# jordi-adell/mcarray

Measured on AMD Instinct MI355X. Metric: STFT frames/sec, 8-mic GCC-PHAT + SRP-PHAT(361) + delay-and-sum beamform @48kHz/1024-pt, higher is better.
Workload: dtype f32 (SRP operands adaptive); 1 GPU; BASELINE configs[2] geometry (8-mic ULA 0.04 m, 48 kHz, N=1024, hop 512, 361 angles, 1 source, no power floor), 8 arrays x 4096 frames per GPU per step; channel rows padded by 64 floats; arrays_per_gpu=8, frames_per_array=4096, srp_precision=adaptive, parallelism=arrays sharded over 1 GPU(s), all_gather of DOA bins+prob

## Files before the change

### mcarray_amd/csrc/api.hip

```cpp
#include "../../include/mcarray_hip.h"
#include "fft1024c.h"
#include "kernels.h"
#include "knobs.h"
#include "stage.h"

#include <chrono>
#include <cmath>
#include <cstdio>
#include <cstdlib>
#include <cstring>
#include <string>
#include <thread>
#include <vector>

using namespace mca;

namespace {

std::string g_create_error;

struct TimedEvent { int id; hipEvent_t a, b; };

}

// ... 1639 lines not shown
           (c->prec == MCA_HIP_SRP_ADAPTIVE || c->prec == MCA_HIP_SRP_FP16) && c->cfg.gcc_weighting != MCA_HIP_GCC_NONE;
}

static int steer_pass_frames(const mca_hip_ctx *c, int n_arrays, int n_frames)
{
    const long long cap = ws_max_bytes(c) / ((long long)n_arrays * STEER_ROW * (long long)sizeof(float2));
    return (int)std::max<long long>(1, std::min<long long>(n_frames, cap));
}

static void steer_policy_begin(mca_hip_ctx *c)
{
    const unsigned long long s = c->steer_seq + 1;
    if (!c->h_steer || c->steer_lost || s <= FB_LAG) return;
    const unsigned long long r = s - FB_LAG;
    if (r <= c->steer_seq_seen) return;
    const unsigned long long *slot = c->h_steer + 2 * ((r - 1) % FB_RING);
    const auto t0 = std::chrono::steady_clock::now();
    while (__atomic_load_n(&slot[1], __ATOMIC_ACQUIRE) != r) {
        if (std::chrono::duration_cast<std::chrono::milliseconds>(std::chrono::steady_clock::now() - t0).count() > FB_WAIT_MS) { c->steer_lost = true; c->steer_spec = true; return; }
        std::this_thread::yield();
    }
    c->steer_seq_seen = r;
    c->steer_spec = __atomic_load_n(&slot[0], __ATOMIC_RELAXED) * STEER_MISS_DEN <= c->steer_call_frames[(r - 1) % FB_RING] * STEER_MISS_NUM;
}

static int steer_prepare(mca_hip_ctx *c, int n_arrays, int n_frames)
{
    if (!c->d_steer_rows) {
        const size_t na = (size_t)c->cfg.max_arrays;
        HIP_TRY(c, hipMalloc((void **)&c->d_steer_rows, (size_t)(c->D + 1) * 4 * 64 * sizeof(float4)));
        HIP_TRY(c, hipMalloc((void **)&c->d_steer_q, (size_t)(c->D + 1) * c->M * 8 * sizeof(float2)));
        HIP_TRY(c, hipMalloc((void **)&c->d_steer_nyq, (size_t)(c->D + 1) * c->M * sizeof(float)));
        HIP_TRY(c, hipMalloc((void **)&c->d_steer_pred, na * sizeof(int)));
        HIP_TRY(c, hipMalloc((void **)&c->d_steer_miss, 3 * sizeof(unsigned long long)));
        if (hipHostMalloc((void **)&c->h_steer, FB_RING * 16, hipHostMallocDefault) == hipSuccess) std::memset(c->h_steer, 0, FB_RING * 16); else { c->h_steer = nullptr; (void)hipGetLastError(); }
        HIP_TRY(c, hipMalloc((void **)&c->d_steer_tail, 2 * na * FFT_H * sizeof(float)));
        HIP_TRY(c, hipMemset(c->d_steer_pred, 0xff, na * sizeof(int)));
        HIP_TRY(c, hipMemset(c->d_steer_miss, 0, 3 * sizeof(unsigned long long)));
        const double unit = (double)c->cfg.sample_rate / (double)FFT_N / 346.1;
        hipLaunchKernelGGL(k_steer_table, dim3(c->D + 1, 4), dim3(64), 0, nullptr, c->d_steer_rows, c->d_steer_q, c->d_steer_nyq, c->d_grid, c->d_micx, c->M, unit);
        HIP_TRY(c, hipGetLastError());
        HIP_TRY(c, hipDeviceSynchronize());
    }
    const size_t rows = (size_t)n_arrays * steer_pass_frames(c, n_arrays, n_frames);
    if (rows > c->steer_Y_rows) {
        HIP_TRY(c, hipDeviceSynchronize());
        if (c->d_steer_Y) (void)hipFree(c->d_steer_Y);
        c->d_steer_Y = nullptr; c->steer_Y_rows = 0;
        HIP_TRY(c, hipMalloc((void **)&c->d_steer_Y, rows * STEER_ROW * sizeof(float2)));
        c->steer_Y_rows = rows;
    }
    return MCA_HIP_OK;
}

static int steer_reserve(mca_hip_ctx *c, int n_arrays, int n_frames) { return steer_applies(c) ? steer_prepare(c, n_arrays, n_frames) : MCA_HIP_OK; }

static int steer_separate(mca_hip_ctx *c, const float *pcm, long long array_stride, long long mic_stride, int n_arrays, int n_frames,
                          const int *doa_bin, float *out_pcm, hipStream_t st)
{
    const size_t a0 = (size_t)c->a0;
    const int pf = steer_pass_frames(c, n_arrays, n_frames);
    const bool fused = c->steer_fused_now && pf == n_frames;
    const size_t smem = (size_t)(F1K_TWORDS + 4 * F1K_SCRATCH) * sizeof(float2);
    float *tails[2] = {c->d_steer_tail, c->d_steer_tail + (size_t)c->cfg.max_arrays * FFT_H};
    time_begin(c, MCA_HIP_K_BEAMFORM, st);
    int pass = 0;
    for (int f0 = 0; f0 < n_frames; f0 += pf, ++pass) {
        const int f1 = std::min(n_frames, f0 + pf), np = f1 - f0;
        const bool last = f1 == n_frames;
        SteerPatchArgs pa{};
        pa.pcm = pcm; pa.array_stride = array_stride; pa.mic_stride = mic_stride; pa.n_arrays = n_arrays; pa.n_frames = n_frames; pa.f0 = f0; pa.f1 = f1;
        pa.window = c->d_window; pa.doa_bin = doa_bin; pa.all = fused ? 0 : 1; pa.miss = c->d_steer_miss;
        pa.bf.rows = c->d_steer_rows; pa.bf.q = c->d_steer_q; pa.bf.nyq = c->d_steer_nyq; pa.bf.pred = c->d_steer_pred + a0; pa.bf.Y = c->d_steer_Y;
        pa.y_f0 = f0; pa.y_frames = fused ? n_frames : np;
        hipLaunchKernelGGL(k_steer_patch, dim3(std::min(STEER_PATCH_WGS, (np + 3) / 4)), dim3(256), smem, st, pa);
        SteerSynthArgs sy{};
        sy.Y = c->d_steer_Y; sy.n_frames = n_frames; sy.f0 = f0; sy.f1 = f1; sy.y_f0 = pa.y_f0; sy.y_frames = pa.y_frames;
        sy.ft = 16;
        while (sy.ft > 2 && (long long)n_arrays * ((np + sy.ft - 1) / sy.ft) < 1024) sy.ft >>= 1;
        sy.out = out_pcm;
        sy.tail_in = pass == 0 ? c->d_tail[c->tail_cur] + a0 * FFT_H : tails[(pass - 1) & 1];
        sy.tail_out = last ? c->d_tail[c->tail_cur ^ 1] + a0 * FFT_H : tails[pass & 1];
        sy.doa_bin = doa_bin; sy.pred_out = last ? c->d_steer_pred + a0 : nullptr;
        if (last && c->h_steer) { sy.report = c->h_steer + 2 * (c->steer_seq % FB_RING); sy.seq = c->steer_seq + 1; sy.miss_total = c->d_steer_miss; }
        const int runs = (np + sy.ft - 1) / sy.ft;
        hipLaunchKernelGGL(k_steer_synth, dim3((runs + 3) / 4, n_arrays), dim3(256), smem, st, sy);
    }
    time_end(c, st);
    HIP_TRY(c, hipGetLastError());
    c->steer_call_frames[c->steer_seq % FB_RING] = (unsigned long long)n_arrays * n_frames; ++c->steer_seq;
    c->steer_frames_total += (unsigned long long)n_arrays * n_frames;
    if (fused) ++c->steer_fused_calls;
    return MCA_HIP_OK;
}

static int separate_impl(mca_hip_ctx *c, const float *pcm, long long array_stride, long long mic_stride,
                         int n_arrays, int n_frames, const float *doa_rad, float *out_pcm, hipStream_t st, const int *doa_bin = nullptr)
{
    const size_t a0 = (size_t)c->a0;
    if (doa_bin && c->d_bftab && c->n2048 && (reinterpret_cast<uintptr_t>(out_pcm) & 7) == 0) {
        BeamformWaveArgs wa{};
        wa.pcm = pcm; wa.array_stride = array_stride; wa.mic_stride = mic_stride;
        wa.M = c->M; wa.n_pairs = c->M; wa.n_frames = n_frames; wa.S = c->S;
        wa.ft = 16;
        for (int ft = 2; ft <= 64; ++ft)
            if ((long long)n_arrays * c->S * ((n_frames + 4 * ft - 2) / (4 * ft - 1)) <= 2LL * c->n_cu) { wa.ft = ft; break; }
        wa.window = c->d_window; wa.doa_bin = doa_bin; wa.table = c->d_bftab; wa.out = out_pcm;
        wa.tail_in = c->d_tail[c->tail_cur] + a0 * c->S * c->H; wa.tail_out = c->d_tail[c->tail_cur ^ 1] + a0 * c->S * c->H;
        const int wgs = (n_frames + 4 * wa.ft - 2) / (4 * wa.ft - 1);
        const size_t smem_w = (size_t)(F1K_TWORDS + 4 * F1K_SCRATCH + 4 * 512) * sizeof(float2);
        time_begin(c, MCA_HIP_K_BEAMFORM, st);
        hipLaunchKernelGGL(k_beamform_wave_2048, dim3(wgs, n_arrays, c->S), dim3(256), smem_w, st, wa);
        time_end(c, st);
        HIP_TRY(c, hipGetLastError());
        return MCA_HIP_OK;
    }
    if (doa_bin && c->d_bftab && wave_beamformer_applies(c)) {
        BeamformWaveArgs wa{};
        wa.pcm = pcm; wa.array_stride = array_stride; wa.mic_stride = mic_stride;
// ... 959 lines not shown
    return MCA_HIP_OK;
}

static int drain_events(mca_hip_ctx *c)
{
    for (auto &e : c->events) {
        HIP_TRY(c, hipEventSynchronize(e.b));
        float ms = 0.f;
        HIP_TRY(c, hipEventElapsedTime(&ms, e.a, e.b));
        c->t_ms[e.id] += ms; c->t_launches[e.id] += 1;
        c->pool.push_back(e.a); c->pool.push_back(e.b);
    }
    c->events.clear();
    return MCA_HIP_OK;
}

int mca_hip_get_timing(mca_hip_ctx *c, int kernel_id, int *launches, double *total_ms)
{
    if (!c || kernel_id < 0 || kernel_id >= MCA_HIP_K_COUNT) return MCA_HIP_ERR_INVALID_ARGUMENT;
    int rc = drain_events(c);
    if (rc) return rc;
    if (launches) *launches = c->t_launches[kernel_id];
    if (total_ms) *total_ms = c->t_ms[kernel_id];
    return MCA_HIP_OK;
}

int mca_hip_reset_timing(mca_hip_ctx *c)
{
    if (!c) return MCA_HIP_ERR_INVALID_ARGUMENT;
    int rc = drain_events(c);
    for (int i = 0; i < MCA_HIP_K_COUNT; ++i) { c->t_ms[i] = 0; c->t_launches[i] = 0; }
    if (c->d_rstats) { HIP_TRY(c, hipDeviceSynchronize()); HIP_TRY(c, hipMemset(c->d_rstats, 0, 32)); }
    c->adapt_frames_total = 0;
    c->fb_groups_prev = 0; c->fb_frames_prev = 0; c->fb_flagged_prev = 0; c->fb_seq_seen = c->fb_calls;
    if (c->fb_state == 2) { c->fb_state = 0; c->adapt_suspended = false; }
    return rc;
}

}
```

### mcarray_amd/csrc/fft1024c.h

```cpp
#pragma once
#include "fft512.h"

namespace mca {

constexpr int F1K_ROW = 18;
constexpr int F1K_SCRATCH = 64 * F1K_ROW;
constexpr int F1K_TWORDS = 64 * F1K_ROW;

__device__ __forceinline__ void f1k_table_init(float2 *tab, int tid, int nthreads)
{
    for (int e = tid; e < 1024; e += nthreads) tab[(e >> 4) * F1K_ROW + (e & 15)] = twiddle(((e >> 4) * (e & 15)) & 1023, 1024, false);
}

__device__ __forceinline__ float2 csub_jb(float2 a, float2 b)
{
    v2f av = to_v2f(a), bv = to_v2f(b), r;
    asm("v_pk_fma_f32 %0, %2, 1.0, %1 op_sel:[1,0,0] op_sel_hi:[0,0,1] neg_hi:[1,0,0]" : "=v"(r) : "v"(av), "v"(bv));
    return from_v2f(r);
}
__device__ __forceinline__ float2 cadd_jb(float2 a, float2 b)
{
    v2f av = to_v2f(a), bv = to_v2f(b), r;
    asm("v_pk_fma_f32 %0, %2, 1.0, %1 op_sel:[1,0,0] op_sel_hi:[0,0,1] neg_lo:[1,0,0]" : "=v"(r) : "v"(av), "v"(bv));
    return from_v2f(r);
}
__device__ __forceinline__ float2 cscale(float2 a, float s)
{
    v2f av = to_v2f(a), sv = {s, s}, r;
    asm("v_pk_mul_f32 %0, %1, %2" : "=v"(r) : "v"(av), "v"(sv));
    return from_v2f(r);
}
__device__ __forceinline__ float2 cmul_mj(float2 a)
{
    v2f av = to_v2f(a), one = {1.f, 1.f}, r;
    asm("v_pk_mul_f32 %0, %1, %2 op_sel:[1,0] op_sel_hi:[0,1] neg_hi:[1,0]" : "=v"(r) : "v"(av), "v"(one));
    return from_v2f(r);
}
__device__ __forceinline__ float2 cmul_pj(float2 a)
{
    v2f av = to_v2f(a), one = {1.f, 1.f}, r;
    asm("v_pk_mul_f32 %0, %1, %2 op_sel:[1,0] op_sel_hi:[0,1] neg_lo:[1,0]" : "=v"(r) : "v"(av), "v"(one));
    return from_v2f(r);
}

template <bool INV>
__device__ __forceinline__ void bfly4(float2 &a0, float2 &a1, float2 &a2, float2 &a3)
{
    const float2 t0 = cadd(a0, a2), t1 = csub(a0, a2), t2 = cadd(a1, a3), t3 = csub(a1, a3);
    a0 = cadd(t0, t2);
    a2 = csub(t0, t2);
    if (!INV) { a1 = csub_jb(t1, t3); a3 = cadd_jb(t1, t3); }
    else { a1 = cadd_jb(t1, t3); a3 = csub_jb(t1, t3); }
}

__device__ __forceinline__ constexpr int dr16(int p) { return (p >> 2) + 4 * (p & 3); }

template <bool INV>
__device__ __forceinline__ void fft16(float2 (&v)[16])
{
    constexpr float R = 0.70710678118654752440f, C1 = 0.92387953251128675613f, S1 = 0.38268343236508977173f;
#pragma unroll
    for (int j = 0; j < 4; ++j) bfly4<INV>(v[j], v[j + 4], v[j + 8], v[j + 12]);
// ... 99 lines not shown
```

### mcarray_amd/csrc/kernels_wave.hip

```cpp
#include <type_traits>

#include "fft1024c.h"
#include "mca_internal.h"
#include "cand_unit.h"
#include "phat_pairs.h"
#include "pair_balance.h"
#include "steer.h"

namespace mca {

__global__ __launch_bounds__(256) void k_bf_table(float2 *tab, const float *grid, const double *mic_x, int M, int n_pairs, double unit)
{
    const int d = blockIdx.x, pr = blockIdx.y;
    const double doa = d == 0 ? 0.0 : (double)grid[d - 1];
    const double cd = cos(doa + 1.57079632679489661923);
    const double sc = 1.0 / ((double)M * 1024.0);
    float2 *row = tab + ((long long)d * n_pairs + pr) * 1024;
    for (int k = threadIdx.x; k < 1024; k += 256) {
        const int kap = k <= 512 ? k : k - 1024;
        double pa[2] = {0.0, 0.0}, pb[2] = {0.0, 0.0};
        for (int e = 0; e < 2; ++e) {
            const int c = 2 * pr + e;
            if (c >= M) continue;
            double turns = (double)kap * (unit * mic_x[c] * cd);
            turns -= rint(turns);
            double sn, cs;
            sincospi(2.0 * turns, &sn, &cs);
            if (k == 512) sn = 0.0;
            (e == 0 ? pa : pb)[0] = cs; (e == 0 ? pa : pb)[1] = sn;
        }
        row[k] = make_float2((float)((pa[0] + pb[1]) * sc), (float)((pa[1] - pb[0]) * sc));
    }
}

__device__ __forceinline__ float2 win_lo(float a, float b, v2f w)
{
    v2f x = {a, b}, r;
    asm("v_pk_mul_f32 %0, %1, %2 op_sel:[0,0] op_sel_hi:[1,0]" : "=v"(r) : "v"(x), "v"(w));
    return from_v2f(r);
}
__device__ __forceinline__ float2 win_hi(float a, float b, v2f w)
{
    v2f x = {a, b}, r;
    asm("v_pk_mul_f32 %0, %2, %1 op_sel:[1,0] op_sel_hi:[1,1]" : "=v"(r) : "v"(x), "v"(w));
    return from_v2f(r);
}

template <bool ODD>
__global__ __launch_bounds__(256, 2) void k_beamform_wave(BeamformWaveArgs p)
{
    constexpr int FOPT = 7;
    extern __shared__ __attribute__((aligned(16))) unsigned char smem_raw[];
    float2 *tab = reinterpret_cast<float2 *>(smem_raw);
    const int tid = threadIdx.x, lane = tid & 63, wave = __builtin_amdgcn_readfirstlane(tid >> 6);
    float2 *buf = tab + F1K_TWORDS + wave * F1K_SCRATCH;
    float *xcarry = reinterpret_cast<float *>(tab + F1K_TWORDS + 4 * F1K_SCRATCH);
    f1k_table_init(tab, tid, 256);
    F1kLane lc;
    lc.init(lane);
    __syncthreads();
    lc.load_t1(tab, lane);

    const int a = p.skew ? blockIdx.x : blockIdx.y;
    const long long as = (long long)a * p.S + blockIdx.z;
    int w0 = (int)blockIdx.x * (4 * p.ft - 1), ft = p.ft;
    if (p.skew) {
        const int g = blockIdx.y, half = gridDim.y >> 1, hi = p.ft + p.skew, lo = p.ft - p.skew;
        ft = g < half ? hi : lo;
        w0 = g < half ? g * (4 * hi - 1) : half * (4 * hi - 1) + (g - half) * (4 * lo - 1);
    }
    const int t0 = wave == 0 ? w0 : w0 + wave * ft - 1;
    const int t1 = min(w0 + (wave + 1) * ft - 1, p.n_frames);
    const bool active = t0 < t1;
    const bool lead_in = wave == 0 && t0 > 0;
    const bool deferred = wave > 0;
    const int tfirst = lead_in ? t0 - 1 : t0;
    const int NP = p.n_pairs;
    float carry[8], first[8];
// ... 536 lines not shown
    const int d = blockIdx.x, pr = blockIdx.y, lane = threadIdx.x, lam = lane <= 32 ? lane : 96 - lane;
    const double doa = d == 0 ? 0.0 : (double)grid[d - 1];
    const double cd = cos(doa + 1.57079632679489661923);
    const double sc = 1.0 / ((double)M * 1024.0);
    auto phasor = [&](int c, int k, double &cs, double &sn) {
        double turns = (double)k * (unit * mic_x[c] * cd);
        turns -= rint(turns);
        sincospi(2.0 * turns, &sn, &cs);
    };
    double ca, sa, cb, sb;
    phasor(2 * pr, lam, ca, sa); phasor(2 * pr + 1, lam, cb, sb);
    rows[((long long)d * gridDim.y + pr) * 64 + lane] = make_float4((float)(ca * sc), (float)(sa * sc), (float)(cb * sc), (float)(sb * sc));
    if (lane < 16) {
        const int c = 2 * pr + (lane >> 3), s = lane & 7;
        double cs, sn;
        phasor(c, 64 * s, cs, sn);
        q[((long long)d * M + c) * 8 + s] = make_float2((float)cs, (float)sn);
    }
    if (lane < 2) {
        double cs, sn;
        phasor(2 * pr + lane, 512, cs, sn);
        nyq[d * M + 2 * pr + lane] = (float)(cs * sc);
    }
}

__global__ __launch_bounds__(256, 2) void k_steer_patch(SteerPatchArgs p)
{
    constexpr int NP = 4, MT = 8;
    extern __shared__ __attribute__((aligned(16))) unsigned char smem_raw[];
    float2 *tab = reinterpret_cast<float2 *>(smem_raw);
    const int tid = threadIdx.x, lane = tid & 63, wave = __builtin_amdgcn_readfirstlane(tid >> 6);
    float2 *buf = tab + F1K_TWORDS + wave * F1K_SCRATCH;
    const int npass = p.f1 - p.f0, stride = 4 * (int)gridDim.x;
    int work = p.all;
    if (!work) {
        for (int a = 0; a < p.n_arrays; ++a) {
            const int pred = p.bf.pred[a];
            for (int fo = (int)blockIdx.x * 4 + wave + stride * lane; fo < npass; fo += stride * 64)
                work |= p.doa_bin[(long long)a * p.n_frames + p.f0 + fo] != pred;
        }
    }
    if (!__syncthreads_or(work)) return;
    f1k_table_init(tab, tid, 256);
    F1kLane lc;
    lc.init(lane);
    __syncthreads();
    const int lam = lane <= 32 ? lane : 96 - lane;
    const bool self = (lane & 31) == 0;
    v2f win[8];
#pragma unroll
    for (int i = 0; i < 8; ++i) { win[i].x = p.window[lane + 128 * i]; win[i].y = p.window[lane + 128 * i + 64]; }
    for (int a = 0; a < p.n_arrays; ++a) {
        const int pred = __builtin_amdgcn_readfirstlane(p.bf.pred[a]);
        const bool every = p.all != 0;
        int missed = 0;
        for (int fo = (int)blockIdx.x * 4 + wave; fo < npass; fo += stride) {
            const int f = p.f0 + fo;
            const int bin = __builtin_amdgcn_readfirstlane(p.doa_bin[(long long)a * p.n_frames + f]);
            if (bin != pred) ++missed;
            else if (!every) continue;
            const float4 *srow = p.bf.rows + (long long)(bin + 1) * (NP * 64);
            const float2 *qrow = p.bf.q + (long long)(bin + 1) * (MT * 8);
            const float *base = p.pcm + (long long)a * p.array_stride + (long long)f * FFT_H;
            float2 *yrow = p.bf.Y + ((long long)a * p.y_frames + f - p.y_f0) * STEER_ROW;
            float xa[16], xb[16];
            auto load_pair = [&](int pr) {
                const float *pa = base + (long long)(2 * pr) * p.mic_stride, *pb = pa + p.mic_stride;
#pragma unroll
                for (int i = 0; i < 16; ++i) { xa[i] = pa[(unsigned)lane + 64 * i]; xb[i] = pb[(unsigned)lane + 64 * i]; }
            };
            load_pair(0);
            float2 Y[8], zn[NP];
#pragma unroll
            for (int pr = 0; pr < NP; ++pr) {
                float2 z[16];
                float4 B;
#pragma unroll
                for (int i = 0; i < 8; ++i) { z[2 * i] = win_lo(xa[2 * i], xb[2 * i], win[i]); z[2 * i + 1] = win_hi(xa[2 * i + 1], xb[2 * i + 1], win[i]); }
                float ma = max3abs(z[0].x, z[1].x, z[2].x), mb = max3abs(z[0].y, z[1].y, z[2].y);
#pragma unroll
                for (int i = 3; i < 15; i += 2) { ma = max3abs(ma, z[i].x, z[i + 1].x); mb = max3abs(mb, z[i].y, z[i + 1].y); }
                ma = max2abs(ma, z[15].x); mb = max2abs(mb, z[15].y);
                const PairBalance pb = pair_balance(ma, mb);
                if (pb.scaled()) {
                    const float sa = pb.sa(), sb = pb.sb();
#pragma unroll
                    for (int i = 0; i < 16; ++i) z[i] = make_float2(z[i].x * sa, z[i].y * sb);
                }
                fft1024c<false, 3>(z, buf, lane, tab, lc, [&]() {
                    B = (srow + pr * 64)[(unsigned)lane];
                    if (pr < NP - 1) load_pair(pr + 1);
                }, lam);
                const float un_a = pb.un_a(), un_b = pb.un_b();
                zn[pr] = make_float2(z[dr16(8)].x * un_a, z[dr16(8)].y * un_b);
                const float4 Bu = steer_base(B, un_a, un_b);
                if (lane == 0) {
                    float2 t[16];
#pragma unroll
                    for (int j = 0; j < 16; ++j) t[j] = z[dr16(j)];
#pragma unroll
                    for (int j = 8; j < 16; ++j) z[dr16(j < 12 ? j + 4 : j - 4)] = t[(j + 1) & 15];
                } else if (self) {
#pragma unroll
                    for (int j = 8; j < 12; ++j) { const float2 t = z[dr16(j)]; z[dr16(j)] = z[dr16(j + 4)]; z[dr16(j + 4)] = t; }
                } else {
#pragma unroll
                    for (int j = 8; j < 12; ++j) {
                        float2 &u = z[dr16(j)], &w = z[dr16(j + 4)];
                        swap_rows32(u.x, w.x); swap_rows32(w.x, u.x);
                        swap_rows32(u.y, w.y); swap_rows32(w.y, u.y);
                    }
                }
#pragma unroll
                for (int s = 0; s < 8; ++s) {
                    const float2 zk = z[dr16(s)], zm = z[dr16(15 - s < 12 ? 15 - s + 4 : 15 - s - 4)];
                    const float2 a2 = make_float2(zk.x + zm.x, zk.y - zm.y);
                    const float2 b2 = make_float2(zk.y + zm.y, zm.x - zk.x);
                    const float2 y = pr == 0 ? make_float2(0.f, 0.f) : Y[s];
                    if (s == 0) Y[s] = steer_mac<true>(y, a2, b2, Bu, a2, b2);
                    else Y[s] = steer_mac<false>(y, a2, b2, Bu, qrow[(2 * pr) * 8 + s], qrow[(2 * pr + 1) * 8 + s]);
                }
                wave_lds_fence();
            }
#pragma unroll
            for (int s = 0; s < 8; ++s) yrow[(unsigned)lam + 64 * s] = s == 0 ? steer_dc(Y[s], lane) : Y[s];
            if (lane == 0) yrow[FFT_H] = make_float2(steer_nyquist<NP>(zn, p.bf.nyq + (bin + 1) * MT), 0.f);
        }
        if (missed && lane == 0) { atomicAdd(p.miss, (unsigned long long)missed); if (pred >= 0) atomicAdd(p.miss + 1, (unsigned long long)missed); }
    }
}

__global__ __launch_bounds__(256) void k_steer_synth(SteerSynthArgs p)
{
    extern __shared__ __attribute__((aligned(16))) unsigned char smem_raw[];
    float2 *tab = reinterpret_cast<float2 *>(smem_raw);
    const int tid = threadIdx.x, lane = tid & 63, wave = __builtin_amdgcn_readfirstlane(tid >> 6);
    float2 *buf = tab + F1K_TWORDS + wave * F1K_SCRATCH;
    f1k_table_init(tab, tid, 256);
    F1kLane lc;
    lc.init(lane);
    __syncthreads();
    const int a = blockIdx.y;
    if (p.pred_out && blockIdx.x == 0 && tid == 0) p.pred_out[a] = p.doa_bin[(long long)a * p.n_frames + p.n_frames - 1];
    if (p.report && blockIdx.x == 0 && a == 0 && tid == 0) {
        const unsigned long long tot = p.miss_total[1];
        p.report[0] = tot - p.miss_total[2];
        p.miss_total[2] = tot;
        __hip_atomic_store(&p.report[1], p.seq, __ATOMIC_RELEASE, __HIP_MEMORY_SCOPE_SYSTEM);
    }
    const int t0 = p.f0 + ((int)blockIdx.x * 4 + wave) * p.ft, t1 = min(t0 + p.ft, p.f1);
    if (t0 >= t1) return;
    const float2 *Yb = p.Y + ((long long)a * p.y_frames - p.y_f0) * STEER_ROW;
    float *ob = p.out + (long long)a * p.n_frames * FFT_H;
    float carry[8];
    if (t0 == p.f0) {
#pragma unroll
        for (int i = 0; i < 8; ++i) carry[i] = p.tail_in[(long long)a * FFT_H + lane + 64 * i];
    }
    int t = t0 > p.f0 ? t0 - 1 : t0;
    float2 yv[8], nv[8];
    float yn, nn = 0.f;
#pragma unroll
    for (int i = 0; i < 8; ++i) yv[i] = Yb[(long long)t * STEER_ROW + (unsigned)lane + 64 * i];
    yn = Yb[(long long)t * STEER_ROW + FFT_H].x;
    for (; t < t1; ++t) {
        float2 y[16];
        steer_inverse(y, yv, yn, buf, lane, tab, lc, [&]() {
            if (t + 1 < t1) {
#pragma unroll
                for (int i = 0; i < 8; ++i) nv[i] = Yb[(long long)(t + 1) * STEER_ROW + (unsigned)lane + 64 * i];
                nn = Yb[(long long)(t + 1) * STEER_ROW + FFT_H].x;
            }
        });
        if (t >= t0) {
#pragma unroll
            for (int i = 0; i < 8; ++i) ob[(long long)t * FFT_H + (unsigned)lane + 64 * i] = carry[i] + y[dr16(i)].x;
        }
#pragma unroll
        for (int i = 0; i < 8; ++i) { carry[i] = y[dr16(i + 8)].x; yv[i] = nv[i]; }
        yn = nn;
    }
    if (t1 == p.f1) {
#pragma unroll
        for (int i = 0; i < 8; ++i) p.tail_out[(long long)a * FFT_H + lane + 64 * i] = carry[i];
    }
}

typedef _Float16 h2 __attribute__((ext_vector_type(2)));
__device__ __forceinline__ h2 rot_j_conj(h2 b)
{
    h2 r;
    const unsigned c = 0x3C00BC00u;
    asm("v_pk_mul_f16 %0, %1, %2 op_sel:[1,0] op_sel_hi:[0,1]" : "=v"(r) : "v"(b), "v"(c));
    return r;
}

template <bool POWER>
__global__ __launch_bounds__(256, 2) void k_stft_phat_wave16(StftPhatArgs p)
{
    constexpr int MT = 16, NP = 8;
    extern __shared__ __attribute__((aligned(16))) unsigned char smem_raw[];
    float2 *tab = reinterpret_cast<float2 *>(smem_raw);
    const int tid = threadIdx.x, lane = tid & 63, wave = __builtin_amdgcn_readfirstlane(tid >> 6);
    float2 *buf = tab + F1K_TWORDS + wave * F1K_SCRATCH;
    float *wtab = reinterpret_cast<float *>(tab + F1K_TWORDS + 4 * F1K_SCRATCH);
    const int fpa = p.fpb + p.skew;
    float2 *nyq = reinterpret_cast<float2 *>(wtab + 1024) + wave * (fpa * NP);
    float2 *nref = reinterpret_cast<float2 *>(wtab + 1024) + 4 * (fpa * NP) + wave * (fpa * NP);
    float *dcbad = reinterpret_cast<float *>(reinterpret_cast<float2 *>(wtab + 1024) + 8 * (fpa * NP)) + wave * fpa;
    constexpr float UNSURE = 1e-10f;
    for (int e = tid; e < 1024; e += 256) wtab[(e & 63) * 16 + (e >> 6)] = p.window[e];
    f1k_table_init(tab, tid, 256);
    F1kLane lc;
    lc.init(lane);
    __syncthreads();
    const int lam = lane <= 32 ? lane : 96 - lane;
    const unsigned voff = (unsigned)lam * 4u;
// ... 173 lines not shown
```

### mcarray_amd/csrc/mca_internal.h

```cpp
#pragma once
#include <hip/hip_runtime.h>

#define MCA_MAX_SOURCES 4
#define MCA_MAX_MICS 16

namespace mca {

constexpr int MK_NB = 4;
constexpr int MK_WARM = 8;
constexpr int BF_NB = 4;
constexpr int GCC2_DOAWARM = 64;
constexpr int SCAN_WARM = 96;
constexpr int KG = 513;
#ifndef MCA_SCAN_CHUNK
#define MCA_SCAN_CHUNK 32
#endif
#ifndef MCA_SCAN_SUB
#define MCA_SCAN_SUB 32
#endif
constexpr int SCAN_CHUNK = MCA_SCAN_CHUNK;
constexpr int SCAN_SUB = MCA_SCAN_SUB;
#ifndef MCA_SCAN_LD
#define MCA_SCAN_LD 8
#endif
// ... 10 lines not shown
struct CandArgs {
    const void *A;
    const void *B;
    int Kp, Dp, a_row_elems;
    const int *list; const int *n_list; int list0, pass_rows;
    unsigned *umask; int umask_words;
    int *need;
    int groups_per_array, n_frames;
    float *C; int c_planes; long long c_plane_stride;
    float *hist_C; int hist_base;
};

constexpr int STEER_QWORDS = 8 * 7;
constexpr int STEER_LDS_ROWS = 13;
constexpr int STEER_Y_ZN = 8, STEER_Y_BASE = 11;
constexpr int STEER_MISS_NUM = 1, STEER_MISS_DEN = 3;
constexpr int STEER_ROW = 520;
struct SteerArgs {
    const float4 *rows;
    const float2 *q;
    const float *nyq;
    const int *pred;
    float2 *Y;
};
constexpr int STEER_PATCH_WGS = 512;
struct SteerPatchArgs {
    const float *pcm; long long array_stride, mic_stride;
    int n_arrays, n_frames;
    int f0, f1;
    const float *window;
    const int *doa_bin;
    SteerArgs bf;
    int y_f0, y_frames;
    int all;
    unsigned long long *miss;
};
struct SteerSynthArgs {
    const float2 *Y; int n_frames, f0, f1, ft, y_f0, y_frames;
    float *out;
    const float *tail_in; float *tail_out;
    const int *doa_bin; int *pred_out;
    unsigned long long *report; unsigned long long seq; unsigned long long *miss_total;
};

struct StftPhatArgs {
    const float *pcm;
    long long array_stride, mic_stride;
    int M, n_frames, frame0, fpb;
    const float *window;
    void *A;
    int Kp;
    int a_row_elems;
    int a_planes;
    float *power;
    int total_frames;
    int N, logH, kg, ula;
    const float2 *tw;
    const int *list; const int *n_list; int list0, list_cap, groups_per_array;
    float *hist_out; const float *hist_in; int hist_base;
    const unsigned short *mrank; int n_merged;
    int no_phat;
    int skew;
    unsigned char *dead;
    unsigned char *unsure;
    int cand_on; CandArgs cand;
    SteerArgs bf;
};

__device__ __forceinline__ void store_a(float *row, const StftPhatArgs &, int cidx, float2 v)
{
    reinterpret_cast<float2 *>(row)[cidx] = v;
}

typedef _Float16 half2_t __attribute__((ext_vector_type(2)));

// ... 322 lines not shown
```

### mcarray_amd/csrc/steer.h

```cpp
#pragma once
#include "fft1024c.h"

namespace mca {

__device__ __forceinline__ float4 steer_base(float4 B, float un_a, float un_b)
{
    const float2 a = cscale(make_float2(B.x, B.y), un_a), b = cscale(make_float2(B.z, B.w), un_b);
    return make_float4(a.x, a.y, b.x, b.y);
}
template <bool FIRST>
__device__ __forceinline__ float2 steer_mac(float2 y, float2 a2, float2 b2, float4 B, float2 qa, float2 qb)
{
    if (!FIRST) { a2 = cmul(a2, qa); b2 = cmul(b2, qb); }
    y = cmac(y, a2, make_float2(B.x, B.y));
    return cmac(y, b2, make_float2(B.z, B.w));
}
__device__ __forceinline__ float2 steer_dc(float2 y0, int lane) { return cscale(y0, lane == 0 ? 0.5f : 1.f); }

template <int NP>
__device__ __forceinline__ float steer_nyquist(const float2 (&zn)[NP], const float *pn)
{
    float yn = 0.f;
#pragma unroll
    for (int pr = 0; pr < NP; ++pr) yn = fmaf(zn[pr].y, pn[2 * pr + 1], fmaf(zn[pr].x, pn[2 * pr], yn));
    return yn;
}

template <typename Mid = F1kNoMid>
__device__ __forceinline__ void steer_inverse(float2 (&y)[16], const float2 (&yv)[8], float yn, float2 *buf, int lane, const float2 *tab, const F1kLane &lc, Mid mid = Mid())
{
#pragma unroll
    for (int i = 0; i < 8; ++i) { y[i] = yv[i]; y[i + 8] = make_float2(0.f, 0.f); }
    fft1024c<true, 3>(y, buf, lane, tab, lc, mid);
    const float sn = (lane & 1) ? -yn : yn;
#pragma unroll
    for (int i = 0; i < 16; ++i) y[i].x += sn;
}

}
```

Baseline: 56.91 million frames/s.

## Fuse mispredicted-frame steering patch into synthesis kernel, drop separate patch launch

In the fused path, the steered-spectrum patch for frames whose DOA bin differs from the prediction now runs inside the synthesis kernel instead of a separate k_steer_patch launch. A ballot over the frame's bins marks the misses, and each missed frame is recomputed inline before its inverse FFT. Cross-wave overlap-add at run boundaries is deferred through LDS, and a last-block atomic counter handles pred/report writes. This removes one kernel launch and its early-exit scan per pass, in exchange for more LDS, extra synchronisation, and register pressure under launch_bounds(256,2).

```diff
diff --git a/mcarray_amd/csrc/api.hip b/mcarray_amd/csrc/api.hip
--- a/mcarray_amd/csrc/api.hip
+++ b/mcarray_amd/csrc/api.hip
@@ -1695,11 +1695,11 @@
         HIP_TRY(c, hipMalloc((void **)&c->d_steer_q, (size_t)(c->D + 1) * c->M * 8 * sizeof(float2)));
         HIP_TRY(c, hipMalloc((void **)&c->d_steer_nyq, (size_t)(c->D + 1) * c->M * sizeof(float)));
         HIP_TRY(c, hipMalloc((void **)&c->d_steer_pred, na * sizeof(int)));
-        HIP_TRY(c, hipMalloc((void **)&c->d_steer_miss, 3 * sizeof(unsigned long long)));
+        HIP_TRY(c, hipMalloc((void **)&c->d_steer_miss, STEER_MISS_WORDS * sizeof(unsigned long long)));
         if (hipHostMalloc((void **)&c->h_steer, FB_RING * 16, hipHostMallocDefault) == hipSuccess) std::memset(c->h_steer, 0, FB_RING * 16); else { c->h_steer = nullptr; (void)hipGetLastError(); }
         HIP_TRY(c, hipMalloc((void **)&c->d_steer_tail, 2 * na * FFT_H * sizeof(float)));
         HIP_TRY(c, hipMemset(c->d_steer_pred, 0xff, na * sizeof(int)));
-        HIP_TRY(c, hipMemset(c->d_steer_miss, 0, 3 * sizeof(unsigned long long)));
+        HIP_TRY(c, hipMemset(c->d_steer_miss, 0, STEER_MISS_WORDS * sizeof(unsigned long long)));
         const double unit = (double)c->cfg.sample_rate / (double)FFT_N / 346.1;
         hipLaunchKernelGGL(k_steer_table, dim3(c->D + 1, 4), dim3(64), 0, nullptr, c->d_steer_rows, c->d_steer_q, c->d_steer_nyq, c->d_grid, c->d_micx, c->M, unit);
         HIP_TRY(c, hipGetLastError());
@@ -1731,23 +1731,28 @@
     for (int f0 = 0; f0 < n_frames; f0 += pf, ++pass) {
         const int f1 = std::min(n_frames, f0 + pf), np = f1 - f0;
         const bool last = f1 == n_frames;
-        SteerPatchArgs pa{};
-        pa.pcm = pcm; pa.array_stride = array_stride; pa.mic_stride = mic_stride; pa.n_arrays = n_arrays; pa.n_frames = n_frames; pa.f0 = f0; pa.f1 = f1;
-        pa.window = c->d_window; pa.doa_bin = doa_bin; pa.all = fused ? 0 : 1; pa.miss = c->d_steer_miss;
-        pa.bf.rows = c->d_steer_rows; pa.bf.q = c->d_steer_q; pa.bf.nyq = c->d_steer_nyq; pa.bf.pred = c->d_steer_pred + a0; pa.bf.Y = c->d_steer_Y;
-        pa.y_f0 = f0; pa.y_frames = fused ? n_frames : np;
-        hipLaunchKernelGGL(k_steer_patch, dim3(std::min(STEER_PATCH_WGS, (np + 3) / 4)), dim3(256), smem, st, pa);
+        SteerArgs bf{};
+        bf.rows = c->d_steer_rows; bf.q = c->d_steer_q; bf.nyq = c->d_steer_nyq; bf.pred = c->d_steer_pred + a0; bf.Y = c->d_steer_Y;
+        const int y_f0 = f0, y_frames = fused ? n_frames : np;
+        if (!fused) {
+            SteerPatchArgs pa{};
+            pa.pcm = pcm; pa.array_stride = array_stride; pa.mic_stride = mic_stride; pa.n_arrays = n_arrays; pa.n_frames = n_frames; pa.f0 = f0; pa.f1 = f1;
+            pa.window = c->d_window; pa.doa_bin = doa_bin; pa.miss = c->d_steer_miss; pa.bf = bf; pa.y_f0 = y_f0; pa.y_frames = y_frames;
+            hipLaunchKernelGGL(k_steer_patch, dim3(std::min(STEER_PATCH_WGS, (np + 3) / 4)), dim3(256), smem, st, pa);
+        }
         SteerSynthArgs sy{};
-        sy.Y = c->d_steer_Y; sy.n_frames = n_frames; sy.f0 = f0; sy.f1 = f1; sy.y_f0 = pa.y_f0; sy.y_frames = pa.y_frames;
+        sy.Y = c->d_steer_Y; sy.n_frames = n_frames; sy.f0 = f0; sy.f1 = f1; sy.y_f0 = y_f0; sy.y_frames = y_frames;
         sy.ft = 16;
         while (sy.ft > 2 && (long long)n_arrays * ((np + sy.ft - 1) / sy.ft) < 1024) sy.ft >>= 1;
         sy.out = out_pcm;
         sy.tail_in = pass == 0 ? c->d_tail[c->tail_cur] + a0 * FFT_H : tails[(pass - 1) & 1];
         sy.tail_out = last ? c->d_tail[c->tail_cur ^ 1] + a0 * FFT_H : tails[pass & 1];
         sy.doa_bin = doa_bin; sy.pred_out = last ? c->d_steer_pred + a0 : nullptr;
-        if (last && c->h_steer) { sy.report = c->h_steer + 2 * (c->steer_seq % FB_RING); sy.seq = c->steer_seq + 1; sy.miss_total = c->d_steer_miss; }
+        if (last && c->h_steer) { sy.report = c->h_steer + 2 * (c->steer_seq % FB_RING); sy.seq = c->steer_seq + 1; }
+        sy.miss = c->d_steer_miss; sy.rows_final = fused ? 0 : 1;
+        sy.pcm = pcm; sy.array_stride = array_stride; sy.mic_stride = mic_stride; sy.window = c->d_window; sy.bf = bf;
         const int runs = (np + sy.ft - 1) / sy.ft;
-        hipLaunchKernelGGL(k_steer_synth, dim3((runs + 3) / 4, n_arrays), dim3(256), smem, st, sy);
+        hipLaunchKernelGGL(k_steer_synth, dim3((runs + 3) / 4, n_arrays), dim3(256), smem + 8 * FFT_H * sizeof(float), st, sy);
     }
     time_end(c, st);
     HIP_TRY(c, hipGetLastError());
@@ -2773,6 +2778,8 @@
     for (int i = 0; i < MCA_HIP_K_COUNT; ++i) { c->t_ms[i] = 0; c->t_launches[i] = 0; }
     if (c->d_rstats) { HIP_TRY(c, hipDeviceSynchronize()); HIP_TRY(c, hipMemset(c->d_rstats, 0, 32)); }
     c->adapt_frames_total = 0;
+    if (c->d_steer_miss) { HIP_TRY(c, hipDeviceSynchronize()); HIP_TRY(c, hipMemset(c->d_steer_miss, 0, STEER_MISS_WORDS * sizeof(unsigned long long))); }
+    c->steer_frames_total = 0; c->steer_fused_calls = 0;
     c->fb_groups_prev = 0; c->fb_frames_prev = 0; c->fb_flagged_prev = 0; c->fb_seq_seen = c->fb_calls;
     if (c->fb_state == 2) { c->fb_state = 0; c->adapt_suspended = false; }
     return rc;
diff --git a/mcarray_amd/csrc/fft1024c.h b/mcarray_amd/csrc/fft1024c.h
--- a/mcarray_amd/csrc/fft1024c.h
+++ b/mcarray_amd/csrc/fft1024c.h
@@ -28,6 +28,18 @@
 {
     v2f av = to_v2f(a), sv = {s, s}, r;
     asm("v_pk_mul_f32 %0, %1, %2" : "=v"(r) : "v"(av), "v"(sv));
+    return from_v2f(r);
+}
+__device__ __forceinline__ float2 win_lo(float a, float b, v2f w)
+{
+    v2f x = {a, b}, r;
+    asm("v_pk_mul_f32 %0, %1, %2 op_sel:[0,0] op_sel_hi:[1,0]" : "=v"(r) : "v"(x), "v"(w));
+    return from_v2f(r);
+}
+__device__ __forceinline__ float2 win_hi(float a, float b, v2f w)
+{
+    v2f x = {a, b}, r;
+    asm("v_pk_mul_f32 %0, %2, %1 op_sel:[1,0] op_sel_hi:[1,1]" : "=v"(r) : "v"(x), "v"(w));
     return from_v2f(r);
 }
 __device__ __forceinline__ float2 cmul_mj(float2 a)
diff --git a/mcarray_amd/csrc/kernels_wave.hip b/mcarray_amd/csrc/kernels_wave.hip
--- a/mcarray_amd/csrc/kernels_wave.hip
+++ b/mcarray_amd/csrc/kernels_wave.hip
@@ -31,19 +31,6 @@
         }
         row[k] = make_float2((float)((pa[0] + pb[1]) * sc), (float)((pa[1] - pb[0]) * sc));
     }
-}
-
-__device__ __forceinline__ float2 win_lo(float a, float b, v2f w)
-{
-    v2f x = {a, b}, r;
-    asm("v_pk_mul_f32 %0, %1, %2 op_sel:[0,0] op_sel_hi:[1,0]" : "=v"(r) : "v"(x), "v"(w));
-    return from_v2f(r);
-}
-__device__ __forceinline__ float2 win_hi(float a, float b, v2f w)
-{
-    v2f x = {a, b}, r;
-    asm("v_pk_mul_f32 %0, %2, %1 op_sel:[1,0] op_sel_hi:[1,1]" : "=v"(r) : "v"(x), "v"(w));
-    return from_v2f(r);
 }
 
 template <bool ODD>
@@ -646,157 +633,148 @@
     const int tid = threadIdx.x, lane = tid & 63, wave = __builtin_amdgcn_readfirstlane(tid >> 6);
     float2 *buf = tab + F1K_TWORDS + wave * F1K_SCRATCH;
     const int npass = p.f1 - p.f0, stride = 4 * (int)gridDim.x;
-    int work = p.all;
-    if (!work) {
-        for (int a = 0; a < p.n_arrays; ++a) {
-            const int pred = p.bf.pred[a];
-            for (int fo = (int)blockIdx.x * 4 + wave + stride * lane; fo < npass; fo += stride * 64)
-                work |= p.doa_bin[(long long)a * p.n_frames + p.f0 + fo] != pred;
-        }
-    }
-    if (!__syncthreads_or(work)) return;
     f1k_table_init(tab, tid, 256);
     F1kLane lc;
     lc.init(lane);
     __syncthreads();
     const int lam = lane <= 32 ? lane : 96 - lane;
-    const bool self = (lane & 31) == 0;
     v2f win[8];
 #pragma unroll
     for (int i = 0; i < 8; ++i) { win[i].x = p.window[lane + 128 * i]; win[i].y = p.window[lane + 128 * i + 64]; }
     for (int a = 0; a < p.n_arrays; ++a) {
         const int pred = __builtin_amdgcn_readfirstlane(p.bf.pred[a]);
-        const bool every = p.all != 0;
         int missed = 0;
         for (int fo = (int)blockIdx.x * 4 + wave; fo < npass; fo += stride) {
             const int f = p.f0 + fo;
             const int bin = __builtin_amdgcn_readfirstlane(p.doa_bin[(long long)a * p.n_frames + f]);
             if (bin != pred) ++missed;
-            else if (!every) continue;
-            const float4 *srow = p.bf.rows + (long long)(bin + 1) * (NP * 64);
-            const float2 *qrow = p.bf.q + (long long)(bin + 1) * (MT * 8);
-            const float *base = p.pcm + (long long)a * p.array_stride + (long long)f * FFT_H;
             float2 *yrow = p.bf.Y + ((long long)a * p.y_frames + f - p.y_f0) * STEER_ROW;
-            float xa[16], xb[16];
-            auto load_pair = [&](int pr) {
-                const float *pa = base + (long long)(2 * pr) * p.mic_stride, *pb = pa + p.mic_stride;
-#pragma unroll
-                for (int i = 0; i < 16; ++i) { xa[i] = pa[(unsigned)lane + 64 * i]; xb[i] = pb[(unsigned)lane + 64 * i]; }
-            };
-            load_pair(0);
-            float2 Y[8], zn[NP];
-#pragma unroll
-            for (int pr = 0; pr < NP; ++pr) {
-                float2 z[16];
-                float4 B;
-#pragma unroll
-                for (int i = 0; i < 8; ++i) { z[2 * i] = win_lo(xa[2 * i], xb[2 * i], win[i]); z[2 * i + 1] = win_hi(xa[2 * i + 1], xb[2 * i + 1], win[i]); }
-                float ma = max3abs(z[0].x, z[1].x, z[2].x), mb = max3abs(z[0].y, z[1].y, z[2].y);
-#pragma unroll
-                for (int i = 3; i < 15; i += 2) { ma = max3abs(ma, z[i].x, z[i + 1].x); mb = max3abs(mb, z[i].y, z[i + 1].y); }
-                ma = max2abs(ma, z[15].x); mb = max2abs(mb, z[15].y);
-                const PairBalance pb = pair_balance(ma, mb);
-                if (pb.scaled()) {
-                    const float sa = pb.sa(), sb = pb.sb();
-#pragma unroll
-                    for (int i = 0; i < 16; ++i) z[i] = make_float2(z[i].x * sa, z[i].y * sb);
-                }
-                fft1024c<false, 3>(z, buf, lane, tab, lc, [&]() {
-                    B = (srow + pr * 64)[(unsigned)lane];
-                    if (pr < NP - 1) load_pair(pr + 1);
-                }, lam);
-                const float un_a = pb.un_a(), un_b = pb.un_b();
-                zn[pr] = make_float2(z[dr16(8)].x * un_a, z[dr16(8)].y * un_b);
-                const float4 Bu = steer_base(B, un_a, un_b);
-                if (lane == 0) {
-                    float2 t[16];
-#pragma unroll
-                    for (int j = 0; j < 16; ++j) t[j] = z[dr16(j)];
-#pragma unroll
-                    for (int j = 8; j < 16; ++j) z[dr16(j < 12 ? j + 4 : j - 4)] = t[(j + 1) & 15];
-                } else if (self) {
-#pragma unroll
-                    for (int j = 8; j < 12; ++j) { const float2 t = z[dr16(j)]; z[dr16(j)] = z[dr16(j + 4)]; z[dr16(j + 4)] = t; }
-                } else {
-#pragma unroll
-                    for (int j = 8; j < 12; ++j) {
-                        float2 &u = z[dr16(j)], &w = z[dr16(j + 4)];
-                        swap_rows32(u.x, w.x); swap_rows32(w.x, u.x);
-                        swap_rows32(u.y, w.y); swap_rows32(w.y, u.y);
-                    }
-                }
-#pragma unroll
-                for (int s = 0; s < 8; ++s) {
-                    const float2 zk = z[dr16(s)], zm = z[dr16(15 - s < 12 ? 15 - s + 4 : 15 - s - 4)];
-                    const float2 a2 = make_float2(zk.x + zm.x, zk.y - zm.y);
-                    const float2 b2 = make_float2(zk.y + zm.y, zm.x - zk.x);
-                    const float2 y = pr == 0 ? make_float2(0.f, 0.f) : Y[s];
-                    if (s == 0) Y[s] = steer_mac<true>(y, a2, b2, Bu, a2, b2);
-                    else Y[s] = steer_mac<false>(y, a2, b2, Bu, qrow[(2 * pr) * 8 + s], qrow[(2 * pr + 1) * 8 + s]);
-                }
-                wave_lds_fence();
-            }
-#pragma unroll
-            for (int s = 0; s < 8; ++s) yrow[(unsigned)lam + 64 * s] = s == 0 ? steer_dc(Y[s], lane) : Y[s];
-            if (lane == 0) yrow[FFT_H] = make_float2(steer_nyquist<NP>(zn, p.bf.nyq + (bin + 1) * MT), 0.f);
+            float2 Y[8];
+            float yn;
+            steer_frame(Y, yn, p.pcm + (long long)a * p.array_stride + (long long)f * FFT_H, p.mic_stride, win, p.bf.rows + (long long)(bin + 1) * (NP * 64),
+                        p.bf.q + (long long)(bin + 1) * (MT * 8), p.bf.nyq + (bin + 1) * MT, buf, lane, lam, tab, lc);
+#pragma unroll
+            for (int s = 0; s < 8; ++s) yrow[(unsigned)lam + 64 * s] = Y[s];
+            if (lane == 0) yrow[FFT_H] = make_float2(yn, 0.f);
         }
         if (missed && lane == 0) { atomicAdd(p.miss, (unsigned long long)missed); if (pred >= 0) atomicAdd(p.miss + 1, (unsigned long long)missed); }
     }
 }
 
-__global__ __launch_bounds__(256) void k_steer_synth(SteerSynthArgs p)
-{
+__global__ __launch_bounds__(256, 2) void k_steer_synth(SteerSynthArgs p)
+{
+    constexpr int NP = 4, MT = 8;
     extern __shared__ __attribute__((aligned(16))) unsigned char smem_raw[];
     float2 *tab = reinterpret_cast<float2 *>(smem_raw);
     const int tid = threadIdx.x, lane = tid & 63, wave = __builtin_amdgcn_readfirstlane(tid >> 6);
     float2 *buf = tab + F1K_TWORDS + wave * F1K_SCRATCH;
+    float *xcarry = reinterpret_cast<float *>(tab + F1K_TWORDS + 4 * F1K_SCRATCH) + wave * FFT_H + lane;
+    float *xfirst = xcarry + 4 * FFT_H;
     f1k_table_init(tab, tid, 256);
     F1kLane lc;
     lc.init(lane);
     __syncthreads();
     const int a = blockIdx.y;
-    if (p.pred_out && blockIdx.x == 0 && tid == 0) p.pred_out[a] = p.doa_bin[(long long)a * p.n_frames + p.n_frames - 1];
-    if (p.report && blockIdx.x == 0 && a == 0 && tid == 0) {
-        const unsigned long long tot = p.miss_total[1];
-        p.report[0] = tot - p.miss_total[2];
-        p.miss_total[2] = tot;
-        __hip_atomic_store(&p.report[1], p.seq, __ATOMIC_RELEASE, __HIP_MEMORY_SCOPE_SYSTEM);
-    }
     const int t0 = p.f0 + ((int)blockIdx.x * 4 + wave) * p.ft, t1 = min(t0 + p.ft, p.f1);
-    if (t0 >= t1) return;
-    const float2 *Yb = p.Y + ((long long)a * p.y_frames - p.y_f0) * STEER_ROW;
+    const bool active = t0 < t1, deferred = wave > 0;
     float *ob = p.out + (long long)a * p.n_frames * FFT_H;
     float carry[8];
-    if (t0 == p.f0) {
-#pragma unroll
-        for (int i = 0; i < 8; ++i) carry[i] = p.tail_in[(long long)a * FFT_H + lane + 64 * i];
-    }
-    int t = t0 > p.f0 ? t0 - 1 : t0;
-    float2 yv[8], nv[8];
-    float yn, nn = 0.f;
-#pragma unroll
-    for (int i = 0; i < 8; ++i) yv[i] = Yb[(long long)t * STEER_ROW + (unsigned)lane + 64 * i];
-    yn = Yb[(long long)t * STEER_ROW + FFT_H].x;
-    for (; t < t1; ++t) {
-        float2 y[16];
-        steer_inverse(y, yv, yn, buf, lane, tab, lc, [&]() {
-            if (t + 1 < t1) {
-#pragma unroll
-                for (int i = 0; i < 8; ++i) nv[i] = Yb[(long long)(t + 1) * STEER_ROW + (unsigned)lane + 64 * i];
-                nn = Yb[(long long)(t + 1) * STEER_ROW + FFT_H].x;
-            }
-        });
-        if (t >= t0) {
-#pragma unroll
-            for (int i = 0; i < 8; ++i) ob[(long long)t * FFT_H + (unsigned)lane + 64 * i] = carry[i] + y[dr16(i)].x;
-        }
-#pragma unroll
-        for (int i = 0; i < 8; ++i) { carry[i] = y[dr16(i + 8)].x; yv[i] = nv[i]; }
-        yn = nn;
-    }
-    if (t1 == p.f1) {
-#pragma unroll
-        for (int i = 0; i < 8; ++i) p.tail_out[(long long)a * FFT_H + lane + 64 * i] = carry[i];
+#pragma unroll
+    for (int i = 0; i < 8; ++i) carry[i] = 0.f;
+    if (active) {
+        const float2 *Yb = p.Y + ((long long)a * p.y_frames - p.y_f0) * STEER_ROW;
+        const int *bins = p.doa_bin + (long long)a * p.n_frames;
+        if (t0 == p.f0) {
+#pragma unroll
+            for (int i = 0; i < 8; ++i) carry[i] = p.tail_in[(long long)a * FFT_H + lane + 64 * i];
+        }
+        const bool lead_in = !deferred && t0 > p.f0;
+        const int tfirst = lead_in ? t0 - 1 : t0;
+        unsigned long long miss = 0;
+        if (!p.rows_final) {
+            const int pred = __builtin_amdgcn_readfirstlane(p.bf.pred[a]);
+            miss = __ballot(tfirst + lane < t1 && bins[min(tfirst + lane, t1 - 1)] != pred);
+            const int missed = __popcll(lead_in ? miss >> 1 : miss);
+            if (missed && lane == 0) { atomicAdd(p.miss, (unsigned long long)missed); if (pred >= 0) atomicAdd(p.miss + 1, (unsigned long long)missed); }
+        }
+        int t = tfirst;
+        float2 yv[8], nv[8];
+        float yn, nn = 0.f;
+#pragma unroll
+        for (int i = 0; i < 8; ++i) yv[i] = Yb[(long long)t * STEER_ROW + (unsigned)lane + 64 * i];
+        yn = Yb[(long long)t * STEER_ROW + FFT_H].x;
+        for (; t < t1; ++t, miss >>= 1) {
+            if (miss & 1) {
+                const int lam = lane <= 32 ? lane : 96 - lane;
+                const int bin = __builtin_amdgcn_readfirstlane(bins[t]);
+#pragma unroll
+                for (int i = 0; i < 8; ++i) xcarry[64 * i] = carry[i];
+                v2f win[8];
+#pragma unroll
+                for (int i = 0; i < 8; ++i) { win[i].x = p.window[lane + 128 * i]; win[i].y = p.window[lane + 128 * i + 64]; }
+                float2 Y[8];
+                float ynl;
+                steer_frame(Y, ynl, p.pcm + (long long)a * p.array_stride + (long long)t * FFT_H, p.mic_stride, win, p.bf.rows + (long long)(bin + 1) * (NP * 64),
+                            p.bf.q + (long long)(bin + 1) * (MT * 8), p.bf.nyq + (bin + 1) * MT, buf, lane, lam, tab, lc);
+#pragma unroll
+                for (int s = 0; s < 8; ++s) buf[lam + 64 * s] = Y[s];
+                wave_lds_fence();
+#pragma unroll
+                for (int i = 0; i < 8; ++i) { yv[i] = buf[lane + 64 * i]; carry[i] = xcarry[64 * i]; }
+                wave_lds_fence();
+                yn = __int_as_float(__builtin_amdgcn_readfirstlane(__float_as_int(ynl)));
+            }
+            float2 y[16];
+            steer_inverse(y, yv, yn, buf, lane, tab, lc, [&]() {
+                if (t + 1 < t1) {
+#pragma unroll
+                    for (int i = 0; i < 8; ++i) nv[i] = Yb[(long long)(t + 1) * STEER_ROW + (unsigned)lane + 64 * i];
+                    nn = Yb[(long long)(t + 1) * STEER_ROW + FFT_H].x;
+                }
+            });
+            if (t >= t0) {
+                if (deferred && t == t0) {
+#pragma unroll
+                    for (int i = 0; i < 8; ++i) xfirst[64 * i] = y[dr16(i)].x;
+                } else {
+#pragma unroll
+                    for (int i = 0; i < 8; ++i) ob[(long long)t * FFT_H + (unsigned)lane + 64 * i] = carry[i] + y[dr16(i)].x;
+                }
+            }
+#pragma unroll
+            for (int i = 0; i < 8; ++i) { carry[i] = y[dr16(i + 8)].x; yv[i] = nv[i]; }
+            yn = nn;
+        }
+        if (t1 == p.f1) {
+#pragma unroll
+            for (int i = 0; i < 8; ++i) p.tail_out[(long long)a * FFT_H + lane + 64 * i] = carry[i];
+        }
+    }
+#pragma unroll
+    for (int i = 0; i < 8; ++i) xcarry[64 * i] = carry[i];
+    __threadfence();
+    __syncthreads();
+    if (active && deferred) {
+#pragma unroll
+        for (int i = 0; i < 8; ++i) ob[(long long)t0 * FFT_H + (unsigned)lane + 64 * i] = (xcarry - FFT_H)[64 * i] + xfirst[64 * i];
+    }
+    int last = 0;
+    if (tid == 0 && (p.pred_out || p.report)) {
+        __threadfence();
+        last = atomicAdd(p.miss + 3, 1ull) + 1ull == (unsigned long long)gridDim.x * gridDim.y;
+    }
+    if (!__syncthreads_or(last)) return;
+    __threadfence();
+    if (p.pred_out)
+        for (int b = tid; b < (int)gridDim.y; b += 256) p.pred_out[b] = p.doa_bin[(long long)b * p.n_frames + p.n_frames - 1];
+    if (tid == 0) {
+        p.miss[3] = 0;
+        if (p.report) {
+            const unsigned long long tot = __hip_atomic_load(p.miss + 1, __ATOMIC_RELAXED, __HIP_MEMORY_SCOPE_AGENT);
+            p.report[0] = tot - p.miss[2];
+            p.miss[2] = tot;
+            __hip_atomic_store(&p.report[1], p.seq, __ATOMIC_RELEASE, __HIP_MEMORY_SCOPE_SYSTEM);
+        }
     }
 }
 
diff --git a/mcarray_amd/csrc/mca_internal.h b/mcarray_amd/csrc/mca_internal.h
--- a/mcarray_amd/csrc/mca_internal.h
+++ b/mcarray_amd/csrc/mca_internal.h
@@ -66,15 +66,19 @@
     const int *doa_bin;
     SteerArgs bf;
     int y_f0, y_frames;
-    int all;
     unsigned long long *miss;
 };
+constexpr int STEER_MISS_WORDS = 4;
 struct SteerSynthArgs {
     const float2 *Y; int n_frames, f0, f1, ft, y_f0, y_frames;
     float *out;
     const float *tail_in; float *tail_out;
     const int *doa_bin; int *pred_out;
-    unsigned long long *report; unsigned long long seq; unsigned long long *miss_total;
+    unsigned long long *report; unsigned long long seq;
+    unsigned long long *miss;
+    int rows_final;
+    const float *pcm; long long array_stride, mic_stride; const float *window;
+    SteerArgs bf;
 };
 
 struct StftPhatArgs {
diff --git a/mcarray_amd/csrc/steer.h b/mcarray_amd/csrc/steer.h
--- a/mcarray_amd/csrc/steer.h
+++ b/mcarray_amd/csrc/steer.h
@@ -1,5 +1,6 @@
 #pragma once
 #include "fft1024c.h"
+#include "pair_balance.h"
 
 namespace mca {
 
@@ -26,6 +27,75 @@
     return yn;
 }
 
+__device__ __forceinline__ void steer_frame(float2 (&Y)[8], float &yn, const float *base, long long mic_stride, const v2f (&win)[8],
+                                            const float4 *srow, const float2 *qrow, const float *pn, float2 *buf, int lane, int lam,
+                                            const float2 *tab, const F1kLane &lc)
+{
+    constexpr int NP = 4;
+    const bool self = (lane & 31) == 0;
+    float xa[16], xb[16];
+    auto load_pair = [&](int pr) {
+        const float *pa = base + (long long)(2 * pr) * mic_stride, *pb = pa + mic_stride;
+#pragma unroll
+        for (int i = 0; i < 16; ++i) { xa[i] = pa[(unsigned)lane + 64 * i]; xb[i] = pb[(unsigned)lane + 64 * i]; }
+    };
+    load_pair(0);
+    float2 zn[NP];
+#pragma unroll
+    for (int pr = 0; pr < NP; ++pr) {
+        float2 z[16];
+        float4 B;
+#pragma unroll
+        for (int i = 0; i < 8; ++i) { z[2 * i] = win_lo(xa[2 * i], xb[2 * i], win[i]); z[2 * i + 1] = win_hi(xa[2 * i + 1], xb[2 * i + 1], win[i]); }
+        float ma = max3abs(z[0].x, z[1].x, z[2].x), mb = max3abs(z[0].y, z[1].y, z[2].y);
+#pragma unroll
+        for (int i = 3; i < 15; i += 2) { ma = max3abs(ma, z[i].x, z[i + 1].x); mb = max3abs(mb, z[i].y, z[i + 1].y); }
+        ma = max2abs(ma, z[15].x); mb = max2abs(mb, z[15].y);
+        const PairBalance pb = pair_balance(ma, mb);
+        if (pb.scaled()) {
+            const float sa = pb.sa(), sb = pb.sb();
+#pragma unroll
+            for (int i = 0; i < 16; ++i) z[i] = make_float2(z[i].x * sa, z[i].y * sb);
+        }
+        fft1024c<false, 3>(z, buf, lane, tab, lc, [&]() {
+            B = (srow + pr * 64)[(unsigned)lane];
+            if (pr < NP - 1) load_pair(pr + 1);
+        }, lam);
+        const float un_a = pb.un_a(), un_b = pb.un_b();
+        zn[pr] = make_float2(z[dr16(8)].x * un_a, z[dr16(8)].y * un_b);
+        const float4 Bu = steer_base(B, un_a, un_b);
+        if (lane == 0) {
+            float2 t[16];
+#pragma unroll
+            for (int j = 0; j < 16; ++j) t[j] = z[dr16(j)];
+#pragma unroll
+            for (int j = 8; j < 16; ++j) z[dr16(j < 12 ? j + 4 : j - 4)] = t[(j + 1) & 15];
+        } else if (self) {
+#pragma unroll
+            for (int j = 8; j < 12; ++j) { const float2 t = z[dr16(j)]; z[dr16(j)] = z[dr16(j + 4)]; z[dr16(j + 4)] = t; }
+        } else {
+#pragma unroll
+            for (int j = 8; j < 12; ++j) {
+                float2 &u = z[dr16(j)], &w = z[dr16(j + 4)];
+                swap_rows32(u.x, w.x); swap_rows32(w.x, u.x);
+                swap_rows32(u.y, w.y); swap_rows32(w.y, u.y);
+            }
+        }
+#pragma unroll
+        for (int s = 0; s < 8; ++s) {
+            const float2 zk = z[dr16(s)], zm = z[dr16(15 - s < 12 ? 15 - s + 4 : 15 - s - 4)];
+            const float2 a2 = make_float2(zk.x + zm.x, zk.y - zm.y);
+            const float2 b2 = make_float2(zk.y + zm.y, zm.x - zk.x);
+            const float2 y = pr == 0 ? make_float2(0.f, 0.f) : Y[s];
+            if (s == 0) Y[s] = steer_mac<true>(y, a2, b2, Bu, a2, b2);
+            else Y[s] = steer_mac<false>(y, a2, b2, Bu, qrow[(2 * pr) * 8 + s], qrow[(2 * pr + 1) * 8 + s]);
+        }
+        wave_lds_fence();
+    }
+    Y[0] = steer_dc(Y[0], lane);
+    yn = steer_nyquist<NP>(zn, pn);
+}
+
 template <typename Mid = F1kNoMid>
 __device__ __forceinline__ void steer_inverse(float2 (&y)[16], const float2 (&yv)[8], float yn, float2 *buf, int lane, const float2 *tab, const F1kLane &lc, Mid mid = Mid())
 {
```

Result: slower. 50.99 million frames/s (-10.4%).
